# michaelnny/alpha_zero

Measured on AMD Instinct MI355X. Metric: self-play moves/sec (whole node), 9x9 Go @ 200 sims/move, higher is better.
Workload: dtype fp32-class evaluator (f16 hi+lo pairs, 3 MFMA products, fp32 accumulate) / f32-f64 tree

## Files before the change

### alpha_zero_amd/csrc/azsp_hip.hip

```cpp
#include <hip/hip_runtime.h>
#include <stdlib.h>

#include <type_traits>

#include "azsp_impl.h"
#include "az_conv64.h"
#include "az_conv19.h"
#include "az_conv_sp.h"
#include "az_conv_sp17.h"
#include "az_resblock_sp17.h"
#include "az_conv_sp2.h"
#include "az_conv_spg.h"
#include "az_stem_spg.h"

static hipError_t g_last = hipSuccess;
#define AZ_HIP(x) ((g_last = (x)) == hipSuccess ? 0 : -1)

template <int N, int GAME, class Op>
__global__ void __launch_bounds__(256) k_game(const AzCfg c, const AzMem m, const Op op, const int g0, const int g1) {
    __shared__ typename Engine<WaveDev, N, GAME>::SC sc[4];
    const int wave = (int)(threadIdx.x >> 6);
    const int g = g0 + (int)blockIdx.x * 4 + wave;
    if (g >= g1) return;
    Engine<WaveDev, N, GAME> e(c, m, g, sc[wave]);
    op(e);
}

__global__ void __launch_bounds__(256) k_dihedral(const DihedralArgs a, long long total) {
    for (long long t = (long long)blockIdx.x * blockDim.x + threadIdx.x; t < total; t += (long long)gridDim.x * blockDim.x)
        az_dihedral_elem(a, t);
}

__global__ void __launch_bounds__(256) k_replay_gather(const ReplayGatherArgs a, long long total) {
    for (long long t = (long long)blockIdx.x * blockDim.x + threadIdx.x; t < total; t += (long long)gridDim.x * blockDim.x)
        az_replay_gather_elem(a, t);
}

__global__ void __launch_bounds__(256) k_bias_act(const BiasActArgs a) {
    for (long long i = (long long)blockIdx.x * blockDim.x + threadIdx.x; i < a.nvec; i += (long long)gridDim.x * blockDim.x)
        az_bias_act_vec(a, i);
}

__global__ void __launch_bounds__(1024) k_harvest_scan(const int* __restrict__ len, int* __restrict__ ofs, int* __restrict__ counts, int n2, int rot,
                                                        int cap, int max_games) {
    __shared__ int ss[1024], sg[1024], best[2];
    const int t = (int)threadIdx.x, per = (n2 + 1023) / 1024, lo = t * per < n2 ? t * per : n2, hi = lo + per < n2 ? lo + per : n2;
    int s = 0, g = 0;
    for (int i = lo; i < hi; ++i) {
        const int l = len[(i + rot) % n2];
        s += l;
        g += l > 0;
    }
    ss[t] = s;
    sg[t] = g;
    if (t < 2) best[t] = 0;
    __syncthreads();
    for (int d = 1; d < 1024; d <<= 1) {
        const int a = t >= d ? ss[t - d] : 0, b = t >= d ? sg[t - d] : 0;
        __syncthreads();
        ss[t] += a;
        sg[t] += b;
        __syncthreads();
    }
    int mine[2] = {0, 0};
    az_harvest_scan_range(len, ofs, n2, rot, cap, max_games, lo, hi, ss[t] - s, sg[t] - g, mine);
    if (mine[1] > 0) {
        atomicMax(&best[0], mine[0]);
        atomicMax(&best[1], mine[1]);
    }
    __syncthreads();
    if (t < 2) counts[t] = best[t];
}

namespace azb {
void* alloc(size_t n) {
    void* p = nullptr;
    if (AZ_HIP(hipMalloc(&p, n))) return nullptr;
    if (AZ_HIP(hipMemset(p, 0, n))) {
        hipFree(p);
        return nullptr;
    }
    return p;
}
void release(void* p) { (void)hipFree(p); }
int h2d(void* d, const void* s, size_t n, void* st) {
    if (AZ_HIP(hipMemcpyAsync(d, s, n, hipMemcpyHostToDevice, (hipStream_t)st))) return -1;
    return AZ_HIP(hipStreamSynchronize((hipStream_t)st));
}
int d2h(void* d, const void* s, size_t n, void* st) {
    if (AZ_HIP(hipMemcpyAsync(d, s, n, hipMemcpyDeviceToHost, (hipStream_t)st))) return -1;
    return AZ_HIP(hipStreamSynchronize((hipStream_t)st));
}
int zero(void* d, size_t n, void* st) { return AZ_HIP(hipMemsetAsync(d, 0, n, (hipStream_t)st)); }
int sync(void* st) { return AZ_HIP(hipStreamSynchronize((hipStream_t)st)); }
void* host_alloc(size_t n) {
    void* p = nullptr;
    return AZ_HIP(hipHostMalloc(&p, n, hipHostMallocDefault)) ? nullptr : p;
}
void host_release(void* p) { (void)hipHostFree(p); }
int set_device(int dev) {
    int n = 0;
    if (AZ_HIP(hipGetDeviceCount(&n)) || n < 1) return -1;
    return AZ_HIP(hipSetDevice(dev));
}
const char* backend_error() { return hipGetErrorString(g_last); }
template <class K, class... A> static int launch_k(K* kernel, unsigned grid, unsigned block, size_t lds, void* st, const A&... args) {
    hipLaunchKernelGGL(kernel, dim3(grid), dim3(block), lds, (hipStream_t)st, args...);
    return AZ_HIP(hipGetLastError());
}
template <class F> static int with_flag(bool flag, F&& f) { return flag ? f(std::true_type{}) : f(std::false_type{}); }
template <class F> static int with_flag(bool f0, bool f1, F&& f) {
    return with_flag(f0, [&](auto F0) { return with_flag(f1, [&](auto F1) { return f(decltype(F0){}, F1); }); });
}
static int cu_count() {
    static int n_cu = 0;
    if (n_cu == 0) {
        int dev = 0;
        hipDeviceProp_t prop;
        if (hipGetDevice(&dev) != hipSuccess || hipGetDeviceProperties(&prop, dev) != hipSuccess) return -1;
        n_cu = prop.multiProcessorCount > 0 ? prop.multiProcessorCount : 256;
    }
    return n_cu;
}
static int persistent_grid(long long units, int k = 1) {
    const int n_cu = cu_count();
    if (n_cu < 0) return -1;
    const long long slots = n_cu / k > 0 ? n_cu / k : 1;
    return k * (int)(units < slots ? units : slots);
}
template <int N, int GAME, class Op> int launch(const AzCfg& c, const AzMem& m, const Op& op, void* st, int g0, int g1) {
    return launch_k(k_game<N, GAME, Op>, (unsigned)((g1 - g0 + 3) / 4), 256, 0, st, c, m, op, g0, g1);
}
int launch_dihedral(const DihedralArgs& a, long long total, void* st) {
    long long blocks = (total + 255) / 256;
    if (blocks > 2048) blocks = 2048;
    return launch_k(k_dihedral, (unsigned)blocks, 256, 0, st, a, total);
}
int launch_replay_gather(const ReplayGatherArgs& a, long long total, void* st) {
    long long blocks = (total + 255) / 256;
    if (blocks > 256 * 16) blocks = 256 * 16;
    return launch_k(k_replay_gather, (unsigned)blocks, 256, 0, st, a, total);
}
int launch_harvest_scan(const int* len, int* ofs, int* counts, int n2, int rot, int cap, int max_games, void* st) {
    return launch_k(k_harvest_scan, 1, 1024, 0, st, len, ofs, counts, n2, rot, cap, max_games);
}
int launch_bias_act(const BiasActArgs& a, void* st) {
    long long blocks = (a.nvec + 255) / 256;
    if (blocks > 256 * 32) blocks = 256 * 32;
    return launch_k(k_bias_act, (unsigned)blocks, 256, 0, st, a);
}
int launch_conv3x3_tiled(const void* x, const void* w, const float* bias, const void* res, void* y, long long boards, int S, int C,
                         int relu, void* st, int f16) {
    if (f16 && (S != CV_S || C != CV_C)) return 1;
    const auto xb = (const unsigned char*)x, rb = (const unsigned char*)res;
    const auto wb = (const unsigned short*)w;
    const auto yb = (unsigned char*)y;
    if (C == C6_C && (S == 17 || S == 9)) {
        const long long ntiles = S == 17 ? boards : (boards + 2) / 3;
        const int grid = persistent_grid(ntiles);
        if (grid < 0) return -1;
        return with_flag(S == 17, res != nullptr, [&](auto G17, auto RES) {
            return launch_k(k_conv3x3_t64<C6Geo<G17 ? 17 : 9>, RES, 8>, grid, CW_THREADS, 0, st, xb, wb, bias, rb, yb, (int)ntiles, relu);
        });
    }
    if (S == C9_S && C == 256) {
        static const bool two_launch = getenv("AZSP_CONV19_TWO_LAUNCH") != nullptr;
        const int grid = persistent_grid(boards, two_launch ? 4 : 8);
        if (grid < 0) return -1;
        if (x == y || res == y) return 1;
        if (!two_launch) {
            return with_flag(res != nullptr, [&](auto RES) {
                return launch_k(k_conv3x3_op19q<RES>, grid, CW_THREADS, 0, st, xb, wb, bias, rb, yb, (int)boards, relu);
            });
        }
        const int rc = with_flag(res != nullptr, [&](auto RES) {
            return launch_k(k_conv3x3_hb19<RES, 16>, grid, CW_THREADS, 0, st, xb, wb, bias, rb, yb, (int)boards, 0, 1, 256, 0, 32, 0);
        });
        if (rc) return rc;
        return launch_k(k_conv3x3_hb19<true, 16>, grid, CW_THREADS, 0, st, xb, wb, bias, (const unsigned char*)yb, yb, (int)boards, relu, 0, 256, 128, 32, 16);
    }
    if (S != CV_S || C != CV_C) return 1;
    const long long ntiles = (boards + CV_TB - 1) / CV_TB;
    const int grid = persistent_grid(ntiles);
    if (grid < 0) return -1;
    return with_flag(res != nullptr, f16 != 0, [&](auto RES, auto F16) {
        return launch_k(k_conv3x3_tiled<RES, 16, F16>, grid, CW_THREADS, 0, st, xb, wb, bias, rb, yb, (int)ntiles, relu);
    });
}
int launch_resblock_tiled(const void* x, const void* w1, const float* b1, const void* w2, const float* b2, void* y, long long boards, int S, int C,
                          void* st) {
    if (C != C6_C || (S != 17 && S != 9)) return 1;
    const long long ntiles = S == 17 ? boards : (boards + 2) / 3;
    const int grid = persistent_grid(ntiles);
    if (grid < 0) return -1;
    return with_flag(S == 17, [&](auto G17) {
        return launch_k(k_resblock64<C6Geo<G17 ? 17 : 9>>, grid, CW_THREADS, 0, st, (const unsigned char*)x, (const unsigned short*)w1, b1,
                        (const unsigned short*)w2, b2, (unsigned char*)y, (int)ntiles);
    });
}
int launch_stem_tiled(const void* x, const void* w, const float* bias, void* y, long long boards, int S, int C, int pad, int relu, void* st, int f16) {
    if (f16 && (S != CV_S || C != CV_C || pad != 1)) return 1;
    const bool t64 = C == C6_C && ((S == 13 && pad == 3) || (S == 9 && pad == 1)), go19 = S == C9_S && C == 256 && pad == 1;
    if (!t64 && !go19 && (S != CV_S || C != CV_C || pad != 1)) return 1;
    const long long ntiles = t64 ? (S == 13 ? boards : (boards + 2) / 3) : go19 ? boards : (boards + CV_TB - 1) / CV_TB;
    const int grid = persistent_grid(ntiles, go19 ? 4 : 1);
    if (grid < 0) return -1;
    const auto xb = (const unsigned char*)x, nores = (const unsigned char*)nullptr;
    const auto wb = (const unsigned short*)w;
    const auto yb = (unsigned char*)y;
    if (t64)
        return with_flag(S == 13, [&](auto G17) {
            return launch_k(k_conv3x3_t64<C6Geo<G17 ? 17 : 9>, false, 4>, grid, CW_THREADS, 0, st, xb, wb, bias, nores, yb, (int)ntiles, relu);
        });
    if (go19) return launch_k(k_conv3x3_hb19<false, 4>, grid, CW_THREADS, 0, st, xb, wb, bias, nores, yb, (int)boards, relu, 1, 32, 0, 4, 0);
    return with_flag(f16 != 0, [&](auto F16) {
        return launch_k(k_conv3x3_tiled<false, 4, F16>, grid, CW_THREADS, 0, st, xb, wb, bias, nores, yb, (int)ntiles, relu);
    });
}
int launch_head_tiled(const void* x, const float* w, const float* bias, void* pol, void* val, long long boards, int S, int C, int npol, int nval,
                      int pol_stride, int val_stride, void* st, int f16) {
    if (C % 8 || C > 1024 || npol + nval != 3) return 1;
    const long long npos = boards * S * S;
    return with_flag(f16 != 0, [&](auto F16) {
        return launch_k(k_head_tiled<3, F16>, (unsigned)((npos + 255) / 256), 256, 0, st, (const unsigned char*)x, w, bias, (unsigned short*)pol,
                        (unsigned short*)val, npos, npol, C, S * S, cv_tile_boards(S) * S * S, pol_stride, val_stride);
    });
}
template <int T1, int T2, bool F16> static int launch_fc_heads_t(const FcHeadsArgs& a, void* st) {
    return launch_k(k_fc_heads<T1, T2, F16>, (unsigned)((a.boards + 127) / 128), 256, 0, st, (const unsigned short*)a.pol, (const unsigned short*)a.val,
                    (const unsigned short*)a.wp, a.bp, a.ks1, (const unsigned short*)a.w1, a.b1, a.ks2, a.w2, a.b2, a.priors, a.values, a.boards, a.A);
}
int launch_fc_heads(const FcHeadsArgs& a, void* st) {
    const int nt1 = (a.A + 31) / 32, nt2 = (a.F + 31) / 32;
    if (a.f16) return nt1 == 3 && nt2 == 4 ? launch_fc_heads_t<3, 4, true>(a, st) : 1;
    if (nt1 == 3 && nt2 == 2) return launch_fc_heads_t<3, 2, false>(a, st);
    if (nt1 == 3 && nt2 == 4) return launch_fc_heads_t<3, 4, false>(a, st);
    if (nt1 == 6 && nt2 == 2) return launch_fc_heads_t<6, 2, false>(a, st);
    if (nt1 == 6 && nt2 == 4) return launch_fc_heads_t<6, 4, false>(a, st);
    if (nt1 == 12 && nt2 == 8) return launch_fc_heads_t<12, 8, false>(a, st);
    return 1;
}
int launch_tile_layout(const void* src, void* dst, long long boards, int S, int C, int to_tiled, void* st) {
    if (C % 8 || S < 1) return 1;
    const int nch = C / 8, tile_rows = cv_tile_boards(S) * S * S;
    const long long nchunks = boards * S * S * nch;
    return launch_k(k_tile_layout, (unsigned)((nchunks + 255) / 256), 256, 0, st, (const unsigned char*)src, (unsigned char*)dst, nchunks, to_tiled, nch,
                    tile_rows);
}
int launch_split_layout(const void* src, void* dst, long long boards, int S, int C, int to_split, void* st, unsigned* range) {
    if (C % 8 || S < 1) return 1;
    const long long nchunks = boards * S * S * (C / 8);
    return launch_k(k_split_layout, (unsigned)((nchunks + 255) / 256), 256, 0, st, (const unsigned char*)src, (unsigned char*)dst, nchunks, to_split, C / 8,
                    S * S, range);
}
template <bool RES, int NCH, int NCG, bool XLO0 = false>
static int launch_sp(const void* x, const void* w, const float* bias, const void* res, void* y, long long boards, int relu, void* st, unsigned* range) {
    const int grid = persistent_grid(boards, NCG);
    if (grid < 0) return -1;
    return launch_k(k_conv3x3_sp<RES, NCH, NCG, XLO0>, grid, CW_THREADS, 0, st, (const unsigned char*)x, (const _Float16*)w, bias, (const unsigned char*)res,
                    (unsigned char*)y, (int)boards, relu, range);
}
template <bool RES, int NCH, bool XLO0 = false>
static int launch_sp17(const void* x, const void* w, const float* bias, const void* res, void* y, long long boards, int relu, void* st, unsigned* range) {
    const int grid = persistent_grid(boards);
    if (grid < 0) return -1;
    return launch_k(k_conv3x3_sp17<RES, NCH, XLO0>, grid, CW_THREADS, 0, st, (const unsigned char*)x, (const _Float16*)w, bias, (const unsigned char*)res,
                    (unsigned char*)y, (int)boards, relu, range);
}
template <bool RES, int KSUB, int NT, int NJ, int HALVES>
static int launch_spg_t(const void* x, const void* w, const float* bias, const void* res, void* y, long long boards, int S, int C, int relu, void* st,
                        unsigned* range) {
    const long long nct = ((long long)S * S + 15) / 16, items = boards * ((nct + NJ - 1) / NJ) * (C / (16 * NT)), grid = (items + 3) / 4;
    if (grid > 0x7fffffffLL) return 1;
    return launch_k(k_conv3x3_spg<RES, KSUB, NT, NJ, HALVES>, (unsigned)grid, 256, 0, st, (const unsigned char*)x, (const _Float16*)w, bias,
                    (const unsigned char*)(RES ? res : nullptr), (unsigned char*)y, (int)boards, S, C, relu, range);
}
template <bool RES, int KSUB, int NT, int HALVES>
static int launch_spgw_t(const void* x, const void* w, const float* bias, const void* res, void* y, long long boards, int S, int C, int relu, void* st,
                         unsigned* range) {
    const long long nct = ((long long)S * S + 15) / 16, grid = (boards * ((nct + 2) / 3) * (C / (64 * NT)) + 7) / 8 * 8;
    if (grid > 0x7fffffffLL || C % (64 * NT)) return 1;
    return launch_k(k_conv3x3_spgw<RES, KSUB, NT, HALVES>, (unsigned)grid, 256, 0, st, (const unsigned char*)x, (const _Float16*)w, bias,
                    (const unsigned char*)(RES ? res : nullptr), (unsigned char*)y, (int)boards, S, C, relu, range);
}
template <int KSUB, int HALVES>
static int launch_spg_k(const void* x, const void* w, const float* bias, const void* res, void* y, long long boards, int S, int C, int relu, void* st,
                        unsigned* range, bool latency) {
    constexpr int NT = KSUB == 2 ? 1 : 2;
    return with_flag(res != nullptr, [&](auto RES) {
        return latency ? launch_spg_t<RES, KSUB, 1, 2, HALVES>(x, w, bias, res, y, boards, S, C, relu, st, range)
                       : launch_spgw_t<RES, KSUB, NT, HALVES>(x, w, bias, res, y, boards, S, C, relu, st, range);
    });
}
static int launch_spg(const void* x, const void* w, const float* bias, const void* res, void* y, long long boards, int S, int C, int relu, void* st,
                      unsigned* range, bool latency, int halves) {
    if (S < 3 || S > 64 || boards < 1 || boards > 0x7fffffffLL) return 1;
    if (C == 64) return launch_spg_k<2, 1>(x, w, bias, res, y, boards, S, C, relu, st, range, latency);
    if (C == 128)
        return halves == 2 ? launch_spg_k<4, 2>(x, w, bias, res, y, boards, S, C, relu, st, range, latency)
                           : launch_spg_k<4, 1>(x, w, bias, res, y, boards, S, C, relu, st, range, latency);
    if (C == 256) return launch_spg_k<8, 1>(x, w, bias, res, y, boards, S, C, relu, st, range, latency);
    return 1;
}
static constexpr long long SPG_DEFAULT_WAVES = 1024;
static long long& spg_max_waves() {
    static long long n = [] {
        const char* e = getenv("AZSP_SPG_MAX_WAVES");
        const long long v = e ? atoll(e) : SPG_DEFAULT_WAVES;
        return v < 0 ? 0LL : v;
    }();
    return n;
}
static bool small_batch(long long boards, int S, int C) { return boards * ((((long long)S * S + 15) / 16 + 1) / 2) * (C / 16) <= spg_max_waves(); }
long long small_batch_waves(long long n) {
    const long long old = spg_max_waves();
    if (n >= 0) spg_max_waves() = n;
    return old;
}
int launch_conv3x3_split(const void* x, const void* w, const float* bias, const void* res, void* y, long long boards, int S, int C, int relu,
                         void* st, unsigned* range) {
    const bool sp17 = S == Sp17Geo::S && C == 64, sp9 = S == SpGeo9::S && (C == 128 || C == 64), small = small_batch(boards, S, C);
    if (!(sp17 || sp9) || small) return launch_spg(x, w, bias, res, y, boards, S, C, relu, st, range, small, sp9 && C == 128 ? 2 : 1);
    if (sp17)
        return with_flag(res != nullptr, [&](auto RES) { return launch_sp17<RES, 8>(x, w, bias, res, y, boards, relu, st, range); });
    if (C == 64) return with_flag(res != nullptr, [&](auto RES) { return launch_sp<RES, 8, 1>(x, w, bias, res, y, boards, relu, st, range); });
    const int grid = persistent_grid(boards, 2);
    if (grid < 0) return -1;
    return with_flag(res != nullptr, [&](auto RES) {
        return launch_k(k_conv3x3_sp2<RES>, grid, CW_THREADS, 0, st, (const unsigned char*)x, (const _Float16*)w, bias, (const unsigned char*)res,
                        (unsigned char*)y, (int)boards, relu, range);
    });
}
enum Scratch {
    SCRATCH_SPG_BLOCK,
    SCRATCH_SP9_TAIL,
    SCRATCH_COUNT
};
static constexpr long long SPG_SCRATCH_BOARDS = 256;
static void* device_scratch(Scratch which, size_t bytes) {
    static void* buf[SCRATCH_COUNT][16] = {};
    int dev = 0;
    if (hipGetDevice(&dev) != hipSuccess || dev < 0 || dev >= 16) return nullptr;
    if (!buf[which][dev] && AZ_HIP(hipMalloc(&buf[which][dev], bytes))) return nullptr;
    return buf[which][dev];
}
int launch_resblock_split(const void* x, const void* w1, const float* b1, const void* w2, const float* b2, void* y, long long boards, int S, int C,
                          void* st, unsigned* range) {
    if (C != 64 || (S != Sb17::S && S != Sb9::S)) return 1;
    const long long pairs = boards / 2;
    const int grid = persistent_grid(S == Sb9::S ? pairs : boards);
    if (grid < 0) return -1;
    if (small_batch(boards, S, C) && boards <= SPG_SCRATCH_BOARDS) {
        void* mid = device_scratch(SCRATCH_SPG_BLOCK, (size_t)SPG_SCRATCH_BOARDS * 2 * 8 * Sb17::S * Sb17::S * 16);
        if (!mid) return -1;
        const int rc = launch_spg(x, w1, b1, nullptr, mid, boards, S, C, 1, st, range, true, 1);
        if (rc) return rc;
        return launch_spg(mid, w2, b2, x, y, boards, S, C, 1, st, range, true, 1);
    }
    const auto xb = (const unsigned char*)x;
    const auto yb = (unsigned char*)y;
    if (S == Sb17::S) return launch_k(k_resblock_sp<Sb17, 6>, grid, CW_THREADS, 0, st, xb, (const _Float16*)w1, b1, (const _Float16*)w2, b2, yb, (int)boards, range);
    if (pairs > 0 && launch_k(k_resblock_sp<Sb9, 6>, grid, CW_THREADS, 0, st, xb, (const _Float16*)w1, b1, (const _Float16*)w2, b2, yb, (int)pairs, range)) return -1;
    if (!(boards & 1)) return 0;
    void* mid = device_scratch(SCRATCH_SP9_TAIL, (size_t)Sb9::GTILEB);
    if (!mid) return -1;
    const size_t off = (size_t)(boards - 1) * Sb9::GTILEB;
    const int rc = launch_sp<false, 8, 1>(xb + off, w1, b1, nullptr, mid, 1, 1, st, range);
    if (rc) return rc;
    return launch_sp<true, 8, 1>(mid, w2, b2, xb + off, yb + off, 1, 1, st, range);
}
int launch_split_features(const float* src, void* dst, long long boards, int S, int cin, void* st, unsigned* range) {
    if (cin < 1 || cin > 32 || S < 1) return 1;
    const long long nitems = boards * 4 * S * S;
    return launch_k(k_split_features, (unsigned)((nitems + 255) / 256), 256, 0, st, src, (unsigned char*)dst, nitems, cin, S * S, range);
}
template <bool XLO0>
static int launch_stem_spg(const void* x, const void* w, const float* bias, void* y, long long boards, int n, int C, int pad, int relu, void* st,
                           unsigned* range) {
    constexpr int NT = 1, NJ = 2;
    const int off = pad - 1, S = n + 2 * off;
    if ((pad != 1 && pad != 3) || n < 1 || S < 3 || S > 64 || (C != 64 && C != 128 && C != 256) || boards < 1 || boards > 0x7fffffffLL) return 1;
    const long long nct = ((long long)S * S + 15) / 16, items = boards * ((nct + NJ - 1) / NJ) * (C / (16 * NT)), grid = (items + 3) / 4;
    if (grid > 0x7fffffffLL) return 1;
    return launch_k(k_stem_spg<XLO0, NT, NJ>, (unsigned)grid, 256, 0, st, (const unsigned char*)x, (const _Float16*)w, bias, (unsigned char*)y, (int)boards,
                    n, off, C, relu, range);
}
static constexpr bool STEM_SPG_DEFAULT_SMALL = false;
int launch_stem_split(const void* x, const void* w, const float* bias, void* y, long long boards, int S, int C, int pad, int relu, void* st,
                      int x_lo_zero, unsigned* range) {
    const bool sp17 = S == 13 && C == 64 && pad == 3;
    const bool sp9 = S == SpGeo9::S && (C == 128 || C == 64) && pad == 1;
    const bool small = (pad == 1 || pad == 3) && small_batch(boards, S + 2 * (pad - 1), C) && (STEM_SPG_DEFAULT_SMALL || spg_max_waves() > SPG_DEFAULT_WAVES);
    return with_flag(x_lo_zero != 0, [&](auto XLO0) {
        if (!(sp17 || sp9) || small) return launch_stem_spg<XLO0>(x, w, bias, y, boards, S, C, pad, relu, st, range);
        if (sp17) return launch_sp17<false, 4, XLO0>(x, w, bias, nullptr, y, boards, relu, st, range);
        return C == 128 ? launch_sp<false, 4, 2, XLO0>(x, w, bias, nullptr, y, boards, relu, st, range)
                        : launch_sp<false, 4, 1, XLO0>(x, w, bias, nullptr, y, boards, relu, st, range);
    });
}
int split_range_read(const unsigned* rec, unsigned out[2], int reset, void* st) {
    void* p = (void*)rec;
    if (!p && AZ_HIP(hipGetSymbolAddress(&p, HIP_SYMBOL(g_sp_range)))) return -1;
    if (AZ_HIP(hipMemcpyAsync(out, p, 2 * sizeof(unsigned), hipMemcpyDeviceToHost, (hipStream_t)st))) return -1;
    if (reset && AZ_HIP(hipMemsetAsync(p, 0, 2 * sizeof(unsigned), (hipStream_t)st))) return -1;
    return AZ_HIP(hipStreamSynchronize((hipStream_t)st));
}
template <int BPB> static int launch_head_split_bpb(const HeadSplitArgs& a, void* st) {
    const int P2 = a.S * a.S;
    const size_t lds = (size_t)(BPB * (3 * ((P2 + 3) & ~3) + a.A + a.F)) * sizeof(float);
    if (lds > 64 * 1024) return 1;
    return launch_k(k_head_split<BPB>, (unsigned)((a.boards + BPB - 1) / BPB), 256, lds, st, (const unsigned char*)a.x, a.hw, a.hb, a.wp_t, a.bp, a.w1_t, a.b1, a.w2,
                    a.b2, a.priors, a.values, a.boards, a.C, P2, a.A, a.F, a.npol);
}
int launch_head_split(const HeadSplitArgs& a, void* st) {
    if (a.C % 8 || a.npol < 1 || a.npol > 2) return 1;
    return launch_head_split_bpb<4>(a, st);
}
}
```

Baseline: 6904.

## Add paired-board 9x9 C=128 conv kernel packing two boards into MFMA tiles

Adds a new persistent conv3x3 kernel for 9x9 boards with 128 channels that handles two boards at once. A constexpr cell map packs both boards' non-corner positions into ten 16-lane tiles, laid out to avoid LDS bank conflicts, so that edge tiles skip taps falling fully outside the board. The two corner cells are batched across several pairs in a side buffer and finished together. The intent is to cut wasted MFMA work on padded 9x9 tiles, at the cost of a very complex hand-scheduled pipeline and an extra launch of the old kernel for an odd leftover board.

```diff
diff --git a/alpha_zero_amd/csrc/az_conv_sp2p.h b/alpha_zero_amd/csrc/az_conv_sp2p.h
--- /dev/null
+++ b/alpha_zero_amd/csrc/az_conv_sp2p.h
@@ -0,0 +1,478 @@
+#pragma once
+#include "az_conv_sp2.h"
+
+#if defined(__HIPCC__)
+#define SP2P_NB 12
+
+struct Sp2pMap {
+    unsigned char cell[10 * 16];
+};
+constexpr Sp2pMap sp2p_map_table = {{
+     10,  13,  20,  28,  11,  15,  17,  26,  32,  47,  49,  65,  37,  40,  48,  70,
+     12,  14,  22,  50,  21,  29,  33,  38,  51,  57,  62,  67,  56,  59,  60,  69,
+     19,  24,  30,  31,  23,  34,  43,  52,  58,  66,  68,  71,  35,  39,  41,  42,
+      1,   2,   3,   4,  82,  83,  84,  85,  86,  87,  88,  89,   5,   6,   7,   8,
+     16,  25,  44,  46,  97, 106, 125, 127, 134, 136, 142, 145,  53,  55,  61,  64,
+     73,  74,  75,  76, 154, 155, 156, 157, 158, 159, 160, 161,  77,  78,  79,  80,
+      0,   9,  18,  27,  81,  90,  99, 108, 117, 126, 135, 144,  36,  45,  54,  63,
+     91,  94, 101, 109,  92,  96,  98, 107, 113, 128, 130, 146, 118, 121, 129, 151,
+     93,  95, 103, 131, 102, 110, 114, 119, 132, 138, 143, 148, 137, 140, 141, 150,
+    100, 105, 111, 112, 104, 115, 124, 133, 139, 147, 149, 152, 116, 120, 122, 123,
+}};
+constexpr int SP2P_NCT = 10, SP2P_KS = 18;
+constexpr bool sp2p_tap_off(int pos, int tap) {
+    const int yy = pos / SpGeo9::S + tap / 3 - 1, xx = pos % SpGeo9::S + tap % 3 - 1;
+    return yy < 0 || yy >= SpGeo9::S || xx < 0 || xx >= SpGeo9::S;
+}
+constexpr bool sp2p_skip(const Sp2pMap& m, int tile, int tap) {
+    for (int n = 0; n < 16; ++n)
+        if (!sp2p_tap_off(m.cell[tile * 16 + n] % SpGeo9::P2, tap)) return false;
+    return true;
+}
+constexpr int sp2p_skips(const Sp2pMap& m) {
+    int n = 0;
+    for (int t = 0; t < SP2P_NCT; ++t)
+        for (int tap = 0; tap < 9; ++tap) n += sp2p_skip(m, t, tap) ? 1 : 0;
+    return n;
+}
+constexpr bool sp2p_map_complete(const Sp2pMap& m) {
+    bool used[2 * SpGeo9::P2] = {};
+    for (int i = 0; i < SP2P_NCT * 16; ++i) {
+        const int v = m.cell[i];
+        if (v >= 2 * SpGeo9::P2 || v % SpGeo9::P2 == SpGeo9::CORNER || used[v]) return false;
+        used[v] = true;
+    }
+    return true;
+}
+constexpr bool sp2p_map_conflict_free(const Sp2pMap& m) {
+    for (int t = 0; t < SP2P_NCT; ++t) {
+        bool bank[16] = {};
+        for (int n = 0; n < 16; ++n) {
+            const int r = (SpGeo9::cell_of(m.cell[t * 16 + n] % SpGeo9::P2) + ((n >= 4 && n < 12) ? 8 : 0)) & 15;
+            if (bank[r]) return false;
+            bank[r] = true;
+        }
+    }
+    return true;
+}
+constexpr bool sp2p_skips_as_designed(const Sp2pMap& m) {
+    for (int t = 0; t < SP2P_NCT; ++t)
+        for (int tap = 0; tap < 9; ++tap) {
+            const bool want = (t == 3 && tap / 3 == 0) || (t == 5 && tap / 3 == 2) || (t == 6 && tap % 3 == 0);
+            if (sp2p_skip(m, t, tap) != want) return false;
+        }
+    return true;
+}
+static_assert(sp2p_map_complete(sp2p_map_table), "pair map: every position of both boards but the two corners exactly once");
+static_assert(sp2p_map_conflict_free(sp2p_map_table), "pair map: conflict-free lane groups in every tile");
+static_assert(sp2p_skips_as_designed(sp2p_map_table) && sp2p_skips(sp2p_map_table) == 9, "pair map: the three edge tiles skip 3 taps each, 9 of 90 (tile, tap) pairs");
+static __device__ const Sp2pMap sp2p_map = sp2p_map_table;
+
+constexpr int sp2p_j0(int u) { return u == 0 ? 0 : u == 1 ? 3 : u == 2 ? 5 : 8; }
+constexpr int sp2p_nj(int u) { return (u & 1) ? 2 : 3; }
+constexpr bool sp2p_has_end(int u) { return u == 0 || u == 3; }
+struct Sp2pSched {
+    int n;
+    int kstart[SP2P_KS + 1];
+    int live_n[SP2P_KS];
+    unsigned char live[SP2P_KS][3];
+    unsigned char t[324], jl[324], tt[324], prod[324], first[324];
+};
+constexpr Sp2pSched sp2p_sched(int u) {
+    Sp2pSched s = {};
+    const int j0 = sp2p_j0(u), nj = sp2p_nj(u);
+    int first_t[3] = {-1, -1, -1};
+    int n = 0;
+    for (int t = 0; t < SP2P_KS; ++t) {
+        int ln = 0;
+        for (int j = 0; j < nj; ++j)
+            if (!sp2p_skip(sp2p_map_table, j0 + j, t / 2)) {
+                s.live[t][ln++] = (unsigned char)j;
+                if (first_t[j] < 0) first_t[j] = t;
+            }
+        s.live_n[t] = ln;
+        s.kstart[t] = n;
+        for (int r6 = 0; r6 < 6; ++r6)
+            for (int k = 0; k < ln; ++k) {
+                const int j = s.live[t][k];
+                s.t[n] = (unsigned char)t, s.jl[n] = (unsigned char)j, s.tt[n] = (unsigned char)(r6 / 3), s.prod[n] = (unsigned char)(r6 % 3);
+                s.first[n] = first_t[j] == t ? 1 : 0;
+                ++n;
+            }
+    }
+    s.kstart[SP2P_KS] = n, s.n = n;
+    return s;
+}
+template <int U> struct Sp2pU {
+    static constexpr Sp2pSched S = sp2p_sched(U);
+};
+static_assert(Sp2pU<0>::S.n + Sp2pU<1>::S.n + Sp2pU<2>::S.n + Sp2pU<3>::S.n == 972, "MFMAs per wave and pair: 1080 less 9 x 12");
+static_assert(Sp2pU<1>::S.n == 180, "the top tile shares its unit with the never-skipped tile");
+
+template <bool RES, int U> struct Sp2pK {
+    static constexpr int KS = SP2P_KS, S0 = 6, NPIECE = 16;
+    static constexpr int E1 = RES ? 4 : 2, PAIR = 2 * E1 + 8, CT_OPS = 2 * PAIR + 2, P2CT = CT_OPS + 1;
+    static constexpr int PU = (U + 3) & 3, NU = (U + 1) & 3;
+    static constexpr int nj = sp2p_nj(U), j0 = sp2p_j0(U), pnj = sp2p_nj(PU), pj0 = sp2p_j0(PU);
+    static constexpr bool END = sp2p_has_end(U), PRE = !sp2p_has_end(PU);
+    static constexpr int N = Sp2pU<U>::S.n, KLAST = Sp2pU<U>::S.kstart[KS - 1];
+    static constexpr int P1 = 5 * pnj, SBX = S0 + P1 + 1, P2 = pnj * P2CT;
+    static constexpr int AVAIL = (END ? KLAST : N - 4) - (SBX + 1);
+    typedef SpSpread<P2, SBX + 1, AVAIL> SP;
+    static constexpr bool DMA = END;
+    static constexpr int PFIRST = SBX + 3, PSTRIDE = U == 0 ? 9 : 6, PLAST = PFIRST + (NPIECE - 1) * PSTRIDE;
+    static_assert(SP::MAXPER <= 1, "the previous unit's finishing fits this unit's MFMA gaps");
+    static_assert(SBX + 1 < Sp2pU<U>::S.kstart[4] && 2 * nj <= S0, "hand-over early in the unit; residual loads in front of it");
+    static_assert(!DMA || (PLAST + 2 * 6 * nj < KLAST && PFIRST > SBX), "pieces behind the barrier that frees the image, well in front of the end barrier");
+};
+template <bool RES, int U> __host__ __device__ constexpr int sp2p_vm_younger() {
+    typedef Sp2pK<RES, U> K;
+    int n = 0;
+    for (int c = 0; c < K::pnj; ++c)
+        for (int st = 0; st < 2; ++st)
+            if (K::SP::slot_of(c * K::P2CT + K::P2CT - 2 + st) > K::PLAST) ++n;
+    return n;
+}
+
+template <bool RES> __global__ void __launch_bounds__(CW_THREADS, 1)
+k_conv3x3_sp2p(const unsigned char* __restrict__ x, const _Float16* __restrict__ w, const float* __restrict__ bias,
+               const unsigned char* __restrict__ res, unsigned char* __restrict__ y, int npairs, int relu, unsigned* range) {
+    typedef SpGeo9 G;
+    constexpr int C = 128, CIN = 128, NCH = 16, NCG = 2;
+    constexpr int KSUB = 2, KS = SP2P_KS;
+    constexpr int NT = 2;
+    constexpr int NJ0 = 3, NJ1 = 2, R = 2;
+    constexpr int LBLK = G::CELLS * 16, LPLANE = NCH * LBLK, LBUF = 2 * LPLANE;
+    constexpr int GBLK = G::P2 * 16, XPLANE = NCH * GBLK, XTILE = 2 * XPLANE;
+    constexpr int YPLANE = (C / 8) * GBLK, YTILE = 2 * YPLANE;
+    constexpr int NP = (G::CELLS + 63) / 64, SPW = 2 * NCH / 4, NPIECE = NP * SPW;
+    constexpr int NF = NT * 2 * KS;
+    constexpr int NF_A = 64;
+    constexpr int P2CT = Sp2pK<RES, 0>::P2CT, PAIR = Sp2pK<RES, 0>::PAIR, E1 = Sp2pK<RES, 0>::E1, S0 = Sp2pK<RES, 0>::S0;
+    static_assert(NPIECE == Sp2pK<RES, 0>::NPIECE && KS % R == 0, "pieces per image; ring phase");
+    constexpr int SIDE_BOARD = 8 * NCH * 16 + 16, SIDE0 = 2 * LBUF + 16, XB0 = SIDE0 + SP2P_NB * SIDE_BOARD, XBCT = 4 * 1024;
+    __shared__ __attribute__((aligned(1024))) unsigned char lds[XB0 + NJ0 * XBCT];
+    static_assert(XB0 + NJ0 * XBCT <= 160 * 1024 && XB0 % 16 == 0, "LDS budget");
+    const int tid = threadIdx.x, lane = tid & 63, l15 = lane & 15, kg = lane >> 4;
+    const int wave = __builtin_amdgcn_readfirstlane(tid >> 6);
+    const int wa = wave >> 1, wb = wave & 1;
+    const unsigned lds0 = (unsigned)(size_t)(__attribute__((address_space(3))) unsigned char*)lds;
+    int cg, slot, nslot;
+    {
+        const int b = (int)blockIdx.x, nb = (int)gridDim.x;
+        nslot = nb / NCG;
+        if (nb % (8 * NCG) == 0) {
+            const int xcd = b & 7, k = b >> 3;
+            cg = k % NCG;
+            slot = xcd + 8 * (k / NCG);
+        } else {
+            cg = b % NCG;
+            slot = b / NCG;
+        }
+    }
+    for (int i = tid; i < (XB0 + NJ0 * XBCT) / 16; i += CW_THREADS) *(cv_u32x4*)(lds + i * 16) = (cv_u32x4){0u, 0u, 0u, 0u};
+    CV_BARRIER();
+    if (slot >= npairs) return;
+
+    sp_f16x8 wf[NF];
+#pragma unroll
+    for (int f = 0; f < NF; ++f) {
+        const int tt = f / (2 * KS), pl = (f / KS) & 1, st = f % KS;
+        wf[f] = *(const sp_f16x8*)(w + ((size_t)((pl * 9 + st / KSUB) * C + cg * 64 + wa * 32 + ((tt + wb) & 1) * 16 + l15)) * CIN + wb * 64 + (st % KSUB) * 32 + kg * 8);
+    }
+    c6_f32x4 bv;
+#pragma unroll
+    for (int e = 0; e < 4; ++e) bv[e] = bias[cg * 64 + wa * 32 + wb * 16 + 4 * kg + e];
+    const float lo_relu = relu ? 0.0f : -__builtin_inff();
+    const float lo_clamp = relu ? 0.0f : -SP_F16_MAX;
+
+    unsigned dsrc[NP];
+    unsigned long long dmask[NP];
+#pragma unroll
+    for (int i = 0; i < NP; ++i) {
+        const int p = 64 * i + lane < G::CELLS ? G::pos_of_cell(64 * i + lane) : -1;
+        dsrc[i] = (unsigned)((p < 0 ? 0 : p) * 16);
+        dmask[i] = __builtin_amdgcn_ballot_w64(p >= 0);
+    }
+    auto dma_piece = [&](const unsigned char* src, unsigned dstbuf, bool live, int i) {
+        const int c = SPW * wave + i / NP, pc = i % NP;
+        const unsigned long long base = (unsigned long long)(src + (size_t)c * GBLK);
+        const unsigned long long mask = live ? dmask[pc] : 0ull;
+        const unsigned dst = dstbuf + (unsigned)(c * LBLK + pc * 1024);
+        asm volatile("s_mov_b64 exec, %0\n\ts_mov_b32 m0, %1\n\ts_nop 0\n\tglobal_load_lds_dwordx4 %2, %3\n\ts_mov_b64 exec, -1"
+                     :
+                     : "s"(mask), "s"(dst), "v"(dsrc[pc]), "s"(base)
+                     : "memory");
+    };
+    unsigned lmap[SP2P_NCT], omap[SP2P_NCT];
+#pragma unroll
+    for (int j = 0; j < SP2P_NCT; ++j) {
+        const int v = sp2p_map.cell[j * 16 + l15], bd = v >= G::P2 ? 1 : 0, pos = v - bd * G::P2;
+        lmap[j] = (unsigned)(bd * LBUF + (G::PITCH * (pos / G::S) + pos % G::S) * 16 + kg * LBLK + wb * (8 * LBLK));
+        omap[j] = (unsigned)(bd * YTILE + pos * 16 + (kg >> 1) * GBLK + (kg & 1) * 8);
+    }
+    auto out_off = [&](int j) __attribute__((always_inline)) {
+        unsigned v = omap[j];
+        asm volatile("" : "+v"(v));
+        return v;
+    };
+    sp_f16x8 bb[R][2][NJ0];
+    auto load_frag = [&](int j, int jl, int s, int rs, int pl) __attribute__((always_inline)) {
+        const int tap = s / KSUB;
+        const int off = ((tap / 3) * G::PITCH + (tap % 3)) * 16 + (s % KSUB) * (4 * LBLK);
+        bb[rs][pl][jl] = *(const sp_f16x8*)(lds + lmap[j] + off + pl * LPLANE);
+    };
+    {
+        const unsigned char* src = x + (size_t)slot * (2 * XTILE);
+#pragma unroll
+        for (int i = 0; i < NPIECE; ++i) dma_piece(src, lds0, true, i);
+        asm volatile("s_waitcnt vmcnt(0)" ::: "memory");
+        CV_BARRIER();
+        static_assert(Sp2pU<0>::S.live_n[0] == NJ0, "the first k-step of a pair has all of U0's tiles");
+#pragma unroll
+        for (int pl = 0; pl < 2; ++pl)
+#pragma unroll
+            for (int j = 0; j < NJ0; ++j) load_frag(j, j, 0, 0, pl);
+    }
+#pragma unroll
+    for (int f = 0; f < NF; ++f) {
+        if (f < NF_A) asm volatile("" : : "a"(wf[f]));
+        else asm volatile("" : : "v"(wf[f]));
+    }
+    asm volatile("" : : "v"(bv), "v"(lmap[0]), "v"(lmap[SP2P_NCT - 1]), "v"(dsrc[0]), "v"(dsrc[NP - 1]));
+
+    c6_f32x4 accm[2][NJ0][NT], accc[2][NJ0][NT];
+    cv_u32x2 rr[2][NJ0][2];
+#pragma unroll
+    for (int a = 0; a < 2; ++a)
+#pragma unroll
+        for (int j = 0; j < NJ0; ++j) {
+#pragma unroll
+            for (int t = 0; t < NT; ++t) accm[a][j][t] = (c6_f32x4){0.0f, 0.0f, 0.0f, 0.0f}, accc[a][j][t] = (c6_f32x4){0.0f, 0.0f, 0.0f, 0.0f};
+            rr[a][j][0] = (cv_u32x2){0u, 0u}, rr[a][j][1] = (cv_u32x2){0u, 0u};
+        }
+    float evv[2] = {0.0f, 0.0f}, sc[2] = {0.0f, 0.0f}, t0 = 0.0f, mx = 0.0f;
+    unsigned hpk[2] = {0u, 0u}, lpk[2] = {0u, 0u};
+    c6_f32x4 xs = (c6_f32x4){0.0f, 0.0f, 0.0f, 0.0f}, xr = (c6_f32x4){0.0f, 0.0f, 0.0f, 0.0f};
+    unsigned char* const xb_mine = lds + XB0 + wave * 1024 + lane * 16;
+    const unsigned char* const xb_partner = lds + XB0 + (wave ^ 1) * 1024 + lane * 16;
+    auto send_op = [&](int set, int c, int o) {
+        if (o < 4) xs[o] = sp2_fma_f32(accc[set][c][1][o], SP_INV_SCALE, accm[set][c][1][o]);
+        else *(c6_f32x4*)(xb_mine + c * XBCT) = xs;
+    };
+    auto fin_op = [&](int set, int c, int mj, unsigned char* out, sp_gptr out_lo, int o, bool store_ok) {
+        if (o == 0) {
+            xr = *(const c6_f32x4*)(xb_partner + c * XBCT);
+            return;
+        }
+        o -= 1;
+        if (o < 2 * PAIR) {
+            const int pr = o / PAIR, k = o % PAIR;
+            if (k < 2 * E1) {
+                const int ei = k / E1, kk = k % E1, e = 2 * pr + ei;
+                const unsigned rh = pr == 0 ? rr[set][c][0].x : rr[set][c][0].y, rl = pr == 0 ? rr[set][c][1].x : rr[set][c][1].y;
+                if (kk == 0) evv[ei] = fmaf(accc[set][c][0][e], SP_INV_SCALE, accm[set][c][0][e]);
+                else if (kk == 1) evv[ei] = cw_add_f32(evv[ei], xr[e]);
+                else if (RES && kk == 2) t0 = ei == 0 ? sp_mix_join<0>(rh, rl) : sp_mix_join<1>(rh, rl);
+                else if (RES && kk == 3) evv[ei] = cw_add_f32(evv[ei], t0);
+            } else {
+                const int kk = k - 2 * E1;
+                if (kk == 0) mx = sp_max3_abs(mx, evv[0], evv[1]);
+                else if (kk == 1) evv[0] = __builtin_amdgcn_fmed3f(evv[0], lo_clamp, SP_F16_MAX);
+                else if (kk == 2) evv[1] = __builtin_amdgcn_fmed3f(evv[1], lo_clamp, SP_F16_MAX);
+                else if (kk == 3) hpk[pr] = sp_cvt_pk(evv[0], evv[1]);
+                else if (kk == 4) sc[0] = sp_mix_diff<0>(hpk[pr], evv[0]);
+                else if (kk == 5) sc[1] = sp_mix_diff<1>(hpk[pr], evv[1]);
+                else if (kk == 6) lpk[pr] = sp_scale_cvt_lo(sc[0]);
+                else lpk[pr] = sp_scale_cvt_hi(lpk[pr], sc[1]);
+            }
+        } else {
+            const unsigned gq = out_off(mj);
+            if (o == 2 * PAIR) {
+                if (store_ok) *(cv_u32x2*)(out + gq) = (cv_u32x2){hpk[0], hpk[1]};
+            } else if (store_ok) *(__attribute__((address_space(1))) cv_u32x2*)(out_lo + gq) = (cv_u32x2){lpk[0], lpk[1]};
+        }
+    };
+
+    const bool copier = tid < 8 * NCH;
+    int csrc, cdst;
+    {
+        constexpr int KF = NCH / 4;
+        const int c = copier ? tid : 0, ks = c % KF, pl = (c / KF) & 1, tp = (c / (2 * KF)) & 3, g4 = c / (8 * KF);
+        csrc = (pl * NCH + 4 * ks + g4) * LBLK + (G::CELL0 + G::PITCH * (G::S - 2 + (tp >> 1)) + (tp & 1)) * 16;
+        cdst = SIDE0 + c * 16;
+    }
+    cv_u32x4 ctmp = (cv_u32x4){0u, 0u, 0u, 0u};
+
+    int it = 0, cb = 0;
+    unsigned char* yprev = y;
+    sp_gptr yprev_lo = (sp_gptr)(unsigned long long)y;
+    for (int pair = slot; pair < npairs; pair += nslot, ++it) {
+        const bool has_next = pair + nslot < npairs;
+        const unsigned char* bsrc = x + (size_t)pair * (2 * XTILE) + XTILE;
+        const unsigned char* nsrc = x + (size_t)(has_next ? pair + nslot : pair) * (2 * XTILE);
+        const size_t yo = (size_t)pair * (2 * YTILE) + (size_t)(cg * 8 + wa * 4 + wb * 2) * GBLK;
+        const unsigned char* rbase = RES ? res + yo : nullptr;
+        unsigned char* ybase = y + yo;
+        unsigned long long rlo = (unsigned long long)(RES ? res + yo : y + yo) + YPLANE, ylo = (unsigned long long)(y + yo) + YPLANE;
+        asm volatile("" : "+s"(rlo), "+s"(ylo));
+        const sp_gcptr rbase_lo = (sp_gcptr)rlo;
+        const sp_gptr ybase_lo = (sp_gptr)ylo;
+        const bool have_prev = it > 0;
+        auto unit = [&](auto UC) __attribute__((always_inline)) {
+            constexpr int u = decltype(UC)::value, set = u & 1, pset = set ^ 1;
+            typedef Sp2pK<RES, u> K;
+            typedef typename K::SP SP;
+            constexpr int nj = K::nj, j0 = K::j0, pj0 = K::pj0, nj0 = sp2p_j0(K::NU);
+            unsigned char* pout = u == 0 ? yprev : ybase;
+            const sp_gptr pout_lo = u == 0 ? yprev_lo : ybase_lo;
+            const bool pstore = u > 0 || have_prev;
+            cp_for_each([&](auto SC) __attribute__((always_inline)) {
+                constexpr int sl = decltype(SC)::value;
+                constexpr int t = Sp2pU<u>::S.t[sl], jl = Sp2pU<u>::S.jl[sl], tt = Sp2pU<u>::S.tt[sl], prod = Sp2pU<u>::S.prod[sl];
+                constexpr int qi = sl - Sp2pU<u>::S.kstart[t];
+                constexpr bool first = Sp2pU<u>::S.first[sl] != 0;
+                if constexpr (K::END && sl == K::KLAST) {
+                    constexpr int VM_YOUNGER = sp2p_vm_younger<RES, u>();
+                    static_assert(VM_YOUNGER < 63, "vmcnt field");
+                    if (pstore) asm volatile("s_waitcnt vmcnt(%0)" ::"n"(VM_YOUNGER) : "memory");
+                    else asm volatile("s_waitcnt vmcnt(0)" ::: "memory");
+                    CV_BARRIER();
+                }
+                if constexpr (K::PRE && sl == S0 - 1) CV_BARRIER();
+                if constexpr (sl == K::SBX) CV_BARRIER();
+                constexpr int fa = (tt * 2 + (prod == 2 ? 1 : 0)) * KS + t, pl = prod == 1 ? 1 : 0;
+                static_assert(!first || fa < NF_A, "an accumulator's first MFMA reads its weights from the AGPRs");
+                if constexpr (prod == 0) {
+                    if constexpr (first && tt == 0) sp_mfma_ac(accm[set][jl][tt], wf[fa], bb[t % R][pl][jl], bv);
+                    else if constexpr (first) sp_mfma_a0(accm[set][jl][tt], wf[fa], bb[t % R][pl][jl]);
+                    else if constexpr (fa < NF_A) sp_mfma_a(accm[set][jl][tt], wf[fa], bb[t % R][pl][jl]);
+                    else sp_mfma_v(accm[set][jl][tt], wf[fa], bb[t % R][pl][jl]);
+                } else if constexpr (prod == 1) {
+                    if constexpr (first) sp_mfma_a0(accc[set][jl][tt], wf[fa], bb[t % R][pl][jl]);
+                    else if constexpr (fa < NF_A) sp_mfma_a(accc[set][jl][tt], wf[fa], bb[t % R][pl][jl]);
+                    else sp_mfma_v(accc[set][jl][tt], wf[fa], bb[t % R][pl][jl]);
+                } else {
+                    if constexpr (fa < NF_A) sp_mfma_a(accc[set][jl][tt], wf[fa], bb[t % R][pl][jl]);
+                    else sp_mfma_v(accc[set][jl][tt], wf[fa], bb[t % R][pl][jl]);
+                }
+                {
+                    constexpr bool lsame = t + 1 < KS;
+                    constexpr int lu = lsame ? u : K::NU, lt = lsame ? t + 1 : 0, lj0 = lsame ? j0 : nj0;
+                    constexpr int lnj = Sp2pU<lu>::S.live_n[lt];
+                    static_assert(2 * lnj <= 6 * Sp2pU<u>::S.live_n[t], "a fragment per MFMA gap");
+                    if constexpr (qi < 2 * lnj) {
+                        constexpr int ljl = Sp2pU<lu>::S.live[lt][qi % lnj];
+                        load_frag(lj0 + ljl, ljl, lt, (t + 1) % R, qi / lnj);
+                    }
+                }
+                if constexpr (sl >= S0 && sl < S0 + K::P1) send_op(pset, (sl - S0) / 5, (sl - S0) % 5);
+                if constexpr (sl > K::SBX) {
+                    constexpr int o = SP::cum(sl - 1);
+                    if constexpr (o < SP::cum(sl)) fin_op(pset, o / P2CT, pj0 + o / P2CT, pout, pout_lo, o % P2CT, pstore);
+                }
+                if constexpr (RES && sl < 2 * nj) {
+                    constexpr int rj = sl >> 1, rp = sl & 1;
+                    if constexpr (rp == 0) rr[set][rj][rp] = *(const cv_u32x2*)(rbase + out_off(j0 + rj));
+                    else rr[set][rj][rp] = *(const __attribute__((address_space(1))) cv_u32x2*)(rbase_lo + out_off(j0 + rj));
+                }
+                __builtin_amdgcn_sched_barrier(0);
+                if constexpr (K::DMA && sl >= K::PFIRST && sl <= K::PLAST && (sl - K::PFIRST) % K::PSTRIDE == 0) {
+                    if constexpr (u == 0) dma_piece(bsrc, lds0 + LBUF, true, (sl - K::PFIRST) / K::PSTRIDE);
+                    else dma_piece(nsrc, lds0, has_next, (sl - K::PFIRST) / K::PSTRIDE);
+                    __builtin_amdgcn_sched_barrier(0);
+                }
+                if constexpr ((u == 0 || u == 2) && sl == Sp2pU<u>::S.kstart[3] - 1) {
+                    if (copier) ctmp = *(const cv_u32x4*)(lds + csrc + (u == 2 ? LBUF : 0));
+                    __builtin_amdgcn_sched_barrier(0);
+                }
+                if constexpr ((u == 0 || u == 2) && sl == Sp2pU<u>::S.kstart[6] - 1) {
+                    if (copier) *(cv_u32x4*)(lds + cdst + (cb + (u == 2 ? 1 : 0)) * SIDE_BOARD) = ctmp;
+                    __builtin_amdgcn_sched_barrier(0);
+                }
+            }, typename CpMakeSeq<K::N>::type{});
+        };
+        unit(CpInt<0>{});
+        unit(CpInt<1>{});
+        unit(CpInt<2>{});
+        unit(CpInt<3>{});
+        yprev = ybase, yprev_lo = ybase_lo;
+        cb += 2;
+        if (cb == SP2P_NB || !has_next) {
+            const int n_ok = cb, it0 = it - (cb / 2 - 1);
+            c6_f32x4 cm[NT], cc[NT];
+            constexpr int KF = NCH / 4;
+            const unsigned char* sb = lds + SIDE0 + l15 * SIDE_BOARD + kg * (8 * KF * 16);
+            const int nb = l15 < n_ok ? l15 : 0;
+            const size_t board = 2 * ((size_t)slot + (size_t)(it0 + (nb >> 1)) * nslot) + (nb & 1);
+            const size_t co = board * YTILE + (size_t)(cg * 8 + wa * 4 + wb * 2 + (kg >> 1)) * GBLK + G::CORNER * 16 + (kg & 1) * 8;
+            if (RES) {
+                rr[0][0][0] = *(const cv_u32x2*)(res + co);
+                rr[0][0][1] = *(const cv_u32x2*)(res + co + YPLANE);
+            }
+            cp_for_each([&](auto TC) __attribute__((always_inline)) {
+                constexpr int u = decltype(TC)::value, tp = u / KSUB, ks = u % KSUB;
+                constexpr int fw = ((tp >> 1) * 3 + 1 + (tp & 1)) * KSUB + ks;
+                const sp_f16x8 bh = *(const sp_f16x8*)(sb + ((tp * 2 + 0) * KF + wb * KSUB + ks) * 16);
+                const sp_f16x8 bl = *(const sp_f16x8*)(sb + ((tp * 2 + 1) * KF + wb * KSUB + ks) * 16);
+#pragma unroll
+                for (int tt = 0; tt < NT; ++tt) {
+                    const int fh = (tt * 2 + 0) * KS + fw, fl = (tt * 2 + 1) * KS + fw;
+                    if (u == 0 && tt == 0) sp_mfma_ac(cm[tt], wf[fh], bh, bv);
+                    else if (u == 0) sp_mfma_a0(cm[tt], wf[fh], bh);
+                    else if (fh < NF_A) sp_mfma_a(cm[tt], wf[fh], bh);
+                    else sp_mfma_v(cm[tt], wf[fh], bh);
+                    if (u == 0) sp_mfma_a0(cc[tt], wf[fh], bl);
+                    else if (fh < NF_A) sp_mfma_a(cc[tt], wf[fh], bl);
+                    else sp_mfma_v(cc[tt], wf[fh], bl);
+                    if (fl < NF_A) sp_mfma_a(cc[tt], wf[fl], bh);
+                    else sp_mfma_v(cc[tt], wf[fl], bh);
+                }
+                __builtin_amdgcn_sched_barrier(0);
+            }, typename CpMakeSeq<4 * KSUB>::type{});
+            asm volatile("s_nop 15\n\ts_nop 15" : "+v"(cm[0]), "+v"(cc[0]), "+v"(cm[1]), "+v"(cc[1]));
+            c6_f32x4 hs;
+#pragma unroll
+            for (int e = 0; e < 4; ++e) hs[e] = fmaf(cc[1][e], SP_INV_SCALE, cm[1][e]);
+            *(c6_f32x4*)(xb_mine) = hs;
+            CV_BARRIER();
+            const c6_f32x4 hr = *(const c6_f32x4*)(xb_partner);
+            float v[4];
+#pragma unroll
+            for (int e = 0; e < 4; ++e) v[e] = fmaf(cc[0][e], SP_INV_SCALE, cm[0][e]) + hr[e];
+            if (RES) {
+                const cv_u32x2 rh = rr[0][0][0], rl = rr[0][0][1];
+                v[0] += sp_join(sp_lo16(rh.x), sp_lo16(rl.x));
+                v[1] += sp_join(sp_hi16(rh.x), sp_hi16(rl.x));
+                v[2] += sp_join(sp_lo16(rh.y), sp_lo16(rl.y));
+                v[3] += sp_join(sp_hi16(rh.y), sp_hi16(rl.y));
+            }
+            _Float16 h[4], l[4];
+#pragma unroll
+            for (int e = 0; e < 4; ++e) {
+                if (l15 < n_ok) mx = fmaxf(mx, fabsf(v[e]));
+                v[e] = fmaxf(v[e], lo_relu);
+                sp_split(v[e], h[e], l[e]);
+            }
+            if (l15 < n_ok) {
+                *(cv_u32x2*)(y + co) = (cv_u32x2){sp_pack(h[0], h[1]), sp_pack(h[2], h[3])};
+                *(cv_u32x2*)(y + co + YPLANE) = (cv_u32x2){sp_pack(l[0], l[1]), sp_pack(l[2], l[3])};
+            }
+            cb = 0;
+            CV_BARRIER();
+        }
+    }
+    asm volatile("s_nop 15\n\ts_nop 15" : "+v"(accm[1][0][0]), "+v"(accm[1][1][0]), "+v"(accc[1][0][0]), "+v"(accc[1][1][0]), "+v"(accm[1][0][1]), "+v"(accm[1][1][1]),
+                 "+v"(accc[1][0][1]), "+v"(accc[1][1][1]));
+#pragma unroll
+    for (int c = 0; c < NJ1; ++c)
+#pragma unroll
+        for (int o = 0; o < 5; ++o) send_op(1, c, o);
+    CV_BARRIER();
+#pragma unroll
+    for (int c = 0; c < NJ1; ++c)
+#pragma unroll
+        for (int o = 0; o < P2CT; ++o) fin_op(1, c, sp2p_j0(3) + c, yprev, yprev_lo, o, true);
+    sp_range_report(mx, range);
+}
+#endif
diff --git a/alpha_zero_amd/csrc/azsp_hip.hip b/alpha_zero_amd/csrc/azsp_hip.hip
--- a/alpha_zero_amd/csrc/azsp_hip.hip
+++ b/alpha_zero_amd/csrc/azsp_hip.hip
@@ -10,6 +10,7 @@
 #include "az_conv_sp17.h"
 #include "az_resblock_sp17.h"
 #include "az_conv_sp2.h"
+#include "az_conv_sp2p.h"
 #include "az_conv_spg.h"
 #include "az_stem_spg.h"
 
@@ -324,11 +325,16 @@
     if (sp17)
         return with_flag(res != nullptr, [&](auto RES) { return launch_sp17<RES, 8>(x, w, bias, res, y, boards, relu, st, range); });
     if (C == 64) return with_flag(res != nullptr, [&](auto RES) { return launch_sp<RES, 8, 1>(x, w, bias, res, y, boards, relu, st, range); });
-    const int grid = persistent_grid(boards, 2);
-    if (grid < 0) return -1;
+    const long long pairs = boards / 2;
+    const int pgrid = persistent_grid(pairs, 2), grid = persistent_grid(boards - 2 * pairs, 2);
+    if (pgrid < 0 || grid < 0) return -1;
+    const size_t off = (size_t)(2 * pairs) * 2 * 128 * SpGeo9::P2 * 2;
     return with_flag(res != nullptr, [&](auto RES) {
-        return launch_k(k_conv3x3_sp2<RES>, grid, CW_THREADS, 0, st, (const unsigned char*)x, (const _Float16*)w, bias, (const unsigned char*)res,
-                        (unsigned char*)y, (int)boards, relu, range);
+        const auto xb = (const unsigned char*)x, rb = (const unsigned char*)res;
+        const auto yb = (unsigned char*)y;
+        if (pairs > 0 && launch_k(k_conv3x3_sp2p<RES>, pgrid, CW_THREADS, 0, st, xb, (const _Float16*)w, bias, rb, yb, (int)pairs, relu, range)) return -1;
+        if (!(boards & 1)) return 0;
+        return launch_k(k_conv3x3_sp2<RES>, grid, CW_THREADS, 0, st, xb + off, (const _Float16*)w, bias, RES ? rb + off : rb, yb + off, 1, relu, range);
     });
 }
 enum Scratch {
```

Measured after the change: 7216 (median of 6 runs). 4.5% higher.
